# suous/RecNeXt

Measured on AMD Instinct MI355X. Metric: images/sec RecNeXt-M3 224x224 bf16, higher is better.
Workload: dtype bf16

## Files before the change

### include/recnext_amd.h

```cpp
#ifndef RECNEXT_AMD_H
#define RECNEXT_AMD_H

#include <stddef.h>

#ifdef __cplusplus
extern "C" {
#endif

#define RCX_ABI_VERSION 7

enum { RCX_DTYPE_F32 = 0, RCX_DTYPE_BF16 = 1, RCX_DTYPE_F16 = 2 };
enum { RCX_MODE_BILINEAR = 0, RCX_MODE_NEAREST = 1 };
enum { RCX_MAX_LEVEL = 8 };

enum {
    RCX_ERR_BAD_ARG = -1,
    RCX_ERR_UNSUPPORTED = -2,
    RCX_ERR_WORKSPACE = -3
};

int rcx_abi_version(void);
const char* rcx_last_error(void);
void rcx_reload_options(void);

// ... 10 lines not shown
size_t rcx_recconv2d_fwd_workspace_bytes(int N, int C, int H, int W, int level, int k, int dtype);

int rcx_recconv2d_fwd(const void* x, void* y, const float* wpack, const float* bpack,
                      void* workspace, size_t workspace_bytes,
                      int N, int C, int H, int W, int level, int k, int mode, int dtype, void* stream);

int rcx_time_next_launch(void* start_event, void* stop_event);
int rcx_launch_events_pending(void);

size_t rcx_recconv2d_train_saved_bytes(int N, int C, int H, int W, int level, int k);
size_t rcx_recconv2d_bwd_workspace_bytes(int N, int C, int H, int W, int level, int k);
int rcx_recconv2d_fwd_train(const void* x, void* y, const float* wpack, const float* bpack, void* saved, size_t saved_bytes,
                            int N, int C, int H, int W, int level, int k, int mode, int dtype, void* stream);
int rcx_recconv2d_bwd_gy_dtype(int N, int C, int H, int W, int level, int k, int dtype);
const char* rcx_recconv2d_bwd_plan(int N, int C, int H, int W, int level, int k, int dtype);
int rcx_recconv2d_bwd(const void* x, const void* gy, int gy_dtype, const float* wpack, const float* wpack_flipped, const void* saved,
                      void* gx, float* gwpack, float* gbpack, void* const* gw_out, void* const* gb_out, int grad_dtype,
                      void* workspace, size_t workspace_bytes,
                      int N, int C, int H, int W, int level, int k, int mode, int dtype, void* stream);

size_t rcx_recconv2d_bwd_input_workspace_bytes(int N, int C, int H, int W, int level, int k);
int rcx_recconv2d_bwd_input_gy_dtype(int N, int C, int H, int W, int level, int k, int dtype);
const char* rcx_recconv2d_bwd_input_plan(int N, int C, int H, int W, int level, int k, int dtype);
int rcx_recconv2d_bwd_input(const void* gy, int gy_dtype, const float* wpack, const float* wpack_flipped, void* gx,
                            void* workspace, size_t workspace_bytes,
                            int N, int C, int H, int W, int level, int k, int mode, int dtype, void* stream);

int rcx_dwconv2d_fwd(const void* x, void* y, const float* w_kkc, const float* bias,
                     int N, int C, int H, int W, int k, int stride,
                     int in_dtype, int out_dtype, void* stream);

int rcx_dwconv2d_mult2_fwd(const void* x, void* y, const float* w_kkc, const float* bias,
                           int N, int Cin, int H, int W, int k, int stride, int dtype, void* stream);

const char* rcx_upadd_dwconv_fwd_plan(int N, int C, int H, int W, int Hc, int Wc, int k, int mode,
                                      int x_dtype, int coarse_dtype, int out_dtype, int has_coarse);
int rcx_upadd_dwconv_fwd(const void* x, const void* coarse, void* y, const float* w_kkc, const float* bias,
                         int N, int C, int H, int W, int Hc, int Wc, int k, int mode,
                         int x_dtype, int coarse_dtype, int out_dtype, void* stream);

size_t rcx_dwconv2d_bwd_workspace_bytes(int C, int k);
int rcx_dwconv2d_bwd(const void* x, const float* gy, const float* w_kkc, const float* w_flipped_kkc,
                     void* gx, float* gw, float* gb, void* workspace, size_t workspace_bytes,
                     int N, int C, int H, int W, int k, int stride, int x_dtype, void* stream);

size_t rcx_upadd_dwconv_bwd_workspace_bytes(int N, int C, int H, int W, int Hc, int Wc, int k);
int rcx_upadd_dwconv_bwd_gy_dtype(int N, int C, int H, int W, int Hc, int Wc, int k, int dtype);
int rcx_upadd_dwconv_bwd(const void* x, const float* coarse, const void* gy, int gy_dtype, const float* w_kkc, const float* w_flipped_kkc,
                         void* gx, float* gcoarse, float* gw, float* gb, void* workspace, size_t workspace_bytes,
                         int N, int C, int H, int W, int Hc, int Wc, int k, int mode, int dtype, void* stream);

int rcx_dwconv2d_mult2_bwd(const void* x, const float* gy, const float* w_kkc, void* gx, float* gw, float* gb,
                           void* workspace, size_t workspace_bytes, int N, int Cin, int H, int W, int k, int dtype, void* stream);

int rcx_linear_attention_fwd(const void* qpre, const void* kpre, const void* v, const void* pe, void* out,
                             int B, int n, int C, int heads, int dtype, void* stream);
int rcx_linear_attention_pe_fwd(const void* qpre, const void* kpre, const void* v, const float* w_pe_kkc, const float* b_pe, void* out,
                                int B, int H, int W, int C, int heads, int dtype, void* stream);

int rcx_recattn_qkcore_launches(int B, int H, int W, int C, int heads);
size_t rcx_recattn_qkcore_workspace_bytes(int B, int H, int W, int C, int heads);
int rcx_recattn_qkcore_fwd(const float* d, const void* wqk_bf16, const float* bqk, const float* w_pe_kkc, const float* b_pe, float* out,
                           void* workspace, size_t workspace_bytes, int B, int H, int W, int C, int heads, void* stream);

int rcx_recattn_down_qkcore_supported(int B, int H, int W, int C, int heads, int x_dtype);
int rcx_recattn_down_qkcore_fwd(const void* x, const float* w_down_kkc, const float* b_down, const void* wqk_bf16, const float* bqk,
// ... 103 lines not shown
```

### recnext_amd/_lib.py

```python
import ctypes
import os

_HERE = os.path.dirname(os.path.abspath(__file__))
LIB_PATH = os.path.join(_HERE, "lib", "librecnext_amd.so")

DTYPE_F32, DTYPE_BF16, DTYPE_F16 = 0, 1, 2
MODE_BILINEAR, MODE_NEAREST = 0, 1
MODES = {"bilinear": MODE_BILINEAR, "nearest": MODE_NEAREST}
MAX_LEVEL = 8
ERR_BAD_ARG, ERR_UNSUPPORTED, ERR_WORKSPACE = -1, -2, -3
ABI_VERSION = 7

_vp, _i, _sz = ctypes.c_void_p, ctypes.c_int, ctypes.c_size_t

SIGNATURES = {
    "rcx_selftest_d16": (_i, [_vp, _vp, _vp]),
    "rcx_abi_version": (_i, []),
    "rcx_last_error": (ctypes.c_char_p, []),
    "rcx_reload_options": (None, []),
    "rcx_recconv2d_fwd_plan": (ctypes.c_char_p, [_i] * 8),
    "rcx_pack_dw_weight": (_i, [_vp, _vp, _i, _i, _i, _vp]),
    "rcx_pack_bias": (_i, [_vp, _vp, _i, _i, _vp]),
    "rcx_pack_recconv_params": (_i, [_vp, _vp, _vp, _vp, _vp, _i, _i, _i, _i, _vp]),
    "rcx_unpack_recconv_grads": (_i, [_vp, _vp, _i, _i, _i, _vp]),
    "rcx_recconv2d_fwd_workspace_bytes": (_sz, [_i] * 7),
    "rcx_recconv2d_fwd": (_i, [_vp, _vp, _vp, _vp, _vp, _sz] + [_i] * 8 + [_vp]),
    "rcx_time_next_launch": (_i, [_vp, _vp]),
    "rcx_launch_events_pending": (_i, []),
    "rcx_recconv2d_train_saved_bytes": (_sz, [_i] * 6),
    "rcx_recconv2d_bwd_workspace_bytes": (_sz, [_i] * 6),
    "rcx_recconv2d_fwd_train": (_i, [_vp, _vp, _vp, _vp, _vp, _sz] + [_i] * 8 + [_vp]),
    "rcx_recconv2d_bwd_gy_dtype": (_i, [_i] * 7),
    "rcx_recconv2d_bwd_plan": (ctypes.c_char_p, [_i] * 7),
    "rcx_upadd_dwconv_bwd_workspace_bytes": (_sz, [_i] * 7),
    "rcx_upadd_dwconv_bwd_gy_dtype": (_i, [_i] * 8),
    "rcx_upadd_dwconv_bwd": (_i, [_vp, _vp, _vp, _i] + [_vp] * 7 + [_sz] + [_i] * 9 + [_vp]),
    "rcx_recconv2d_bwd": (_i, [_vp, _vp, _i] + [_vp] * 8 + [_i, _vp, _sz] + [_i] * 8 + [_vp]),
    "rcx_recconv2d_bwd_input_workspace_bytes": (_sz, [_i] * 6),
    "rcx_recconv2d_bwd_input_gy_dtype": (_i, [_i] * 7),
    "rcx_recconv2d_bwd_input_plan": (ctypes.c_char_p, [_i] * 7),
    "rcx_recconv2d_bwd_input": (_i, [_vp, _i, _vp, _vp, _vp, _vp, _sz] + [_i] * 8 + [_vp]),
    "rcx_dwconv2d_fwd": (_i, [_vp, _vp, _vp, _vp] + [_i] * 8 + [_vp]),
    "rcx_dwconv2d_mult2_fwd": (_i, [_vp, _vp, _vp, _vp] + [_i] * 7 + [_vp]),
    "rcx_upadd_dwconv_fwd": (_i, [_vp, _vp, _vp, _vp, _vp] + [_i] * 11 + [_vp]),
    "rcx_upadd_dwconv_fwd_plan": (ctypes.c_char_p, [_i] * 12),
    "rcx_linear_attention_pe_fwd": (_i, [_vp] * 6 + [_i] * 6 + [_vp]),
    "rcx_recattn_qkcore_launches": (_i, [_i] * 5),
    "rcx_recattn_qkcore_workspace_bytes": (_sz, [_i] * 5),
    "rcx_recattn_qkcore_fwd": (_i, [_vp] * 7 + [_sz] + [_i] * 5 + [_vp]),
    "rcx_recattn_down_qkcore_supported": (_i, [_i] * 6),
    "rcx_recattn_down_qkcore_fwd": (_i, [_vp] * 8 + [_i] * 6 + [_vp]),
    "rcx_stem_supported": (_i, [_i] * 6),
    "rcx_stem_pack_bytes": (_sz, [_i] * 2),
    "rcx_stem_fwd": (_i, [_vp] * 6 + [_i] * 6 + [_vp]),
    "rcx_stem3_supported": (_i, [_i] * 6),
    "rcx_stem3_pack_bytes": (_sz, [_i] * 2),
    "rcx_stem3_workspace_bytes": (_sz, [_i] * 4),
    "rcx_stem3_fwd": (_i, [_vp] * 9 + [_sz] + [_i] * 6 + [_vp]),
    "rcx_channel_mlp_supported": (_i, [_i] * 4),
    "rcx_channel_mlp_pack_bytes": (_sz, [_i] * 2),
    "rcx_channel_mlp_fwd": (_i, [_vp] * 5 + [_i] * 4 + [_vp]),
    "rcx_recattn2d_fwd_supported": (_i, [_i] * 7),
    "rcx_recattn2d_fwd": (_i, [_vp] * 10 + [_i] * 7 + [_vp]),
    "rcx_dwconv2d_bwd_workspace_bytes": (ctypes.c_size_t, [_i, _i]),
    "rcx_dwconv2d_bwd": (_i, [_vp, _vp, _vp, _vp, _vp, _vp, _vp, _vp, ctypes.c_size_t] + [_i] * 7 + [_vp]),
    "rcx_dwconv2d_mult2_bwd": (_i, [_vp, _vp, _vp, _vp, _vp, _vp, _vp, ctypes.c_size_t] + [_i] * 6 + [_vp]),
    "rcx_linear_attention_fwd": (_i, [_vp, _vp, _vp, _vp, _vp] + [_i] * 5 + [_vp]),
    "rcx_ls_recattn_supported": (_i, [_i] * 7),
    "rcx_ls_recattn_fwd": (_i, [_vp] * 15 + [_i] * 7 + [_vp]),
    "rcx_ls_la3_supported": (_i, [_i] * 7),
    "rcx_ls_la3_fwd": (_i, [_vp] * 11 + [_i] * 7 + [_vp]),
    "rcx_ls_recattn_tiled_supported": (_i, [_i] * 7),
    "rcx_ls_recattn_tiled_workspace_bytes": (_sz, [_i] * 7),
    "rcx_ls_recattn_tiled_fwd": (_i, [_vp] * 16 + [_sz] + [_i] * 7 + [_vp]),
    "rcx_ls_la3_tiled_supported": (_i, [_i] * 7),
    "rcx_ls_la3_tiled_workspace_bytes": (_sz, [_i] * 7),
# ... 59 lines not shown
```

### recnext_amd/csrc/rcx_api.hip

```cpp
#include "../../include/recnext_amd.h"
#include "rcx_opts.h"
#include "rcx_launch.h"

#include <cstdarg>
#include <initializer_list>
#include <cstdio>
#include <cstdlib>

namespace {

thread_local char g_err[512] = "";

int fail(int code, const char* fmt, ...)
{
    va_list ap;
    va_start(ap, fmt);
    vsnprintf(g_err, sizeof(g_err), fmt, ap);
    va_end(ap);
    return code;
}

int hip_fail(hipError_t e, const char* what, const char* prefix = "")
{
    snprintf(g_err, sizeof(g_err), "%s%s: %s", prefix, what, hipGetErrorString(e));
// ... 56 lines not shown

size_t split_bytes(int N, int C, int H, int W) { return 2 * align256(sizeof(float) * (size_t)N * C * (H / 2) * (W / 2)); }

bool use_lanes(int N, int C, int H, int W, int level, int k, int dtype)
{
    return !rcx::opt::hand_kernels_off() && rcx::lanes_applicable(N, C, H, W, level, k, dtype);
}

bool upcpt_everywhere() { return rcx::opt::str(rcx::opt::UPADD_CPT)[0] == 'a'; }

enum StepKernel { STEP_GENERIC, STEP_LANES, STEP_CPT, STEP_CPL14, STEP_CONV5_LANES };

StepKernel pick_dwconv(int N, int C, int H, int W, int k, int stride, int in_dt, int out_dt)
{
    if (rcx::opt::hand_kernels_off()) return STEP_GENERIC;
    if (rcx::down5_cpl7_applicable(N, C, H, W, k, stride, in_dt, out_dt)) return STEP_CPL14;
    const bool lanes_ok = rcx::down5_lanes_applicable(N, C, H, W, k, stride, in_dt, out_dt);
    if (lanes_ok && !upcpt_everywhere() && !(W % 14 != 0 && C % 64 == 0)) return STEP_LANES;
    if (rcx::down5_cpt_applicable(N, C, H, W, k, stride, in_dt, out_dt)) return STEP_CPT;
    if (lanes_ok) return STEP_LANES;
    if (stride == 1 && rcx::conv5_lanes_applicable(N, C, H, W, k, in_dt, out_dt)) return STEP_CONV5_LANES;
    return STEP_GENERIC;
}

StepKernel pick_upadd(int N, int C, int H, int W, int Hc, int Wc, int k, int x_dt, int c_dt, int out_dt, bool has_coarse)
{
    if (rcx::opt::hand_kernels_off()) return STEP_GENERIC;
    if (!has_coarse) return rcx::conv5_lanes_applicable(N, C, H, W, k, x_dt, out_dt) ? STEP_CONV5_LANES : STEP_GENERIC;
    if (rcx::upadd_cpl14_applicable(N, C, H, W, Hc, Wc, k, x_dt, c_dt, out_dt)) return STEP_CPL14;
    const bool lanes_ok = rcx::upadd_lanes_applicable(N, C, H, W, Hc, Wc, k, x_dt, c_dt, out_dt);
    const bool whole = C % 64 == 0 && !(W % 14 != 0 && H < 64);
    if ((whole || !lanes_ok || upcpt_everywhere()) && rcx::upadd_cpt_applicable(N, C, H, W, Hc, Wc, k, x_dt, c_dt, out_dt)) return STEP_CPT;
    return lanes_ok ? STEP_LANES : STEP_GENERIC;
}

enum FwdSchedule { FWD_LANES, FWD_SPLIT, FWD_PLANE, FWD_NESTED, FWD_GENERIC };
FwdSchedule fwd_schedule(int N, int C, int H, int W, int level, int k, int dtype);

bool use_nested(int N, int C, int H, int W, int level, int k, int dtype)
{
    if (rcx::opt::hand_kernels_off() || rcx::opt::off(rcx::opt::NESTED) || level < 1 || k != 5 || (H & 1) || (W & 1)) return false;
    const StepKernel d = pick_dwconv(N, C, H, W, k, 2, dtype, RCX_DTYPE_F32);
    const StepKernel u = pick_upadd(N, C, H, W, H / 2, W / 2, k, dtype, RCX_DTYPE_F32, dtype, true);
    if (d == STEP_GENERIC || u == STEP_GENERIC) return false;
    return fwd_schedule(N, C, H / 2, W / 2, level - 1, k, RCX_DTYPE_F32) != FWD_GENERIC;
}

FwdSchedule fwd_schedule(int N, int C, int H, int W, int level, int k, int dtype)
{
    if (use_lanes(N, C, H, W, level, k, dtype)) return FWD_LANES;
    if (use_split(N, C, H, W, level, k, dtype)) return FWD_SPLIT;
    if (use_plane(N, C, H, W, level, k, dtype)) return FWD_PLANE;
    if (use_nested(N, C, H, W, level, k, dtype)) return FWD_NESTED;
    return FWD_GENERIC;
}

size_t nested_own_bytes(int N, int C, int H, int W) { return 2 * align256(sizeof(float) * (size_t)N * C * (H / 2) * (W / 2)); }

hipError_t step_dwconv(const void* x, void* y, const float* w, const float* b, int N, int C, int H, int W, int k, int stride,
                       int in_dt, int out_dt, hipStream_t s)
{
    switch (pick_dwconv(N, C, H, W, k, stride, in_dt, out_dt)) {
    case STEP_CPL14: return rcx::down5_cpl7(x, y, w, b, N, C, H, in_dt, s);
    case STEP_LANES: return rcx::down5_lanes(x, y, w, b, N, C, H, W, in_dt, out_dt, s);
    case STEP_CPT: return rcx::down5_cpt(x, y, w, b, N, C, H, W, in_dt, out_dt, s);
    case STEP_CONV5_LANES: return rcx::conv5_lanes(x, y, w, b, N, C, H, W, in_dt, s);
// ... 544 lines not shown
    const size_t need = bwd_input_workspace(L, sch.kind);
    if (need && (!workspace || workspace_bytes < need))
        return fail(RCX_ERR_WORKSPACE, "input-backward workspace too small: need %zu bytes, got %zu", need, workspace_bytes);
    if (gy_dtype != RCX_DTYPE_F32 && !(sch.kind != BWD_STEPS && gy_dtype == dtype))
        return fail(RCX_ERR_UNSUPPORTED, "gy of dtype %d: this problem takes float32 (rcx_recconv2d_bwd_input_gy_dtype)", gy_dtype);
    BwdRun B{L, false, "bwd input: "};
    B.gy = gy; B.gx = gx; B.wpack = wpack; B.wflip = wpack_flipped; B.ws = (char*)workspace;
    B.gy_dt = gy_dtype; B.N = N; B.C = C; B.level = level; B.k = k; B.mode = mode; B.dtype = dtype; B.s = (hipStream_t)stream;
    if (sch.kind == BWD_ONE) RCX_TRY(one_launch(B, gy, gy_dtype, gx, 0, H, level, dtype), "fused block", B.prefix);
    else return sch.kind == BWD_TILED ? bwd_tiled(B, sch.m) : bwd_steps(B, sch.m);
    return 0;
}

#undef RCX_TRY

int rcx_dwconv2d_fwd(const void* x, void* y, const float* w_kkc, const float* bias,
                     int N, int C, int H, int W, int k, int stride, int in_dtype, int out_dtype, void* stream)
{
    if (int rc = check_common(x, y, N, C, H, W, k, in_dtype)) return rc;
    if (!known_dtype(out_dtype)) return fail(RCX_ERR_BAD_ARG, "unknown dtype %d", out_dtype);
    if (!w_kkc) return fail(RCX_ERR_BAD_ARG, "null weight");
    if (stride != 1 && stride != 2) return fail(RCX_ERR_UNSUPPORTED, "stride %d not supported (1 or 2)", stride);
    hipError_t e = step_dwconv(x, y, w_kkc, bias, N, C, H, W, k, stride, in_dtype, out_dtype, (hipStream_t)stream);
    return e == hipSuccess ? 0 : hip_fail(e, "rcx_dwconv2d_fwd");
}

int rcx_dwconv2d_mult2_fwd(const void* x, void* y, const float* w_kkc, const float* bias,
                           int N, int Cin, int H, int W, int k, int stride, int dtype, void* stream)
{
    if (int rc = check_common(x, y, N, Cin, H, W, k, dtype)) return rc;
    if (!w_kkc) return fail(RCX_ERR_BAD_ARG, "null weight");
    if (stride != 1 && stride != 2) return fail(RCX_ERR_UNSUPPORTED, "stride %d not supported (1 or 2)", stride);
    hipError_t e;
    const bool lanes_ok = !rcx::opt::hand_kernels_off() && rcx::down_lanes_applicable(N, Cin, H, W, k, stride, dtype);
    const bool tiled_ok = !rcx::opt::hand_kernels_off() && rcx::down7m2_cpt_applicable(N, Cin, H, W, k, stride, dtype);
    if (tiled_ok && (!lanes_ok || H > 64 || W > 64 || (H <= 14 && W <= 14) || upcpt_everywhere()))
        e = rcx::down7m2_cpt(x, y, w_kkc, bias, N, Cin, H, W, dtype, (hipStream_t)stream);
    else if (lanes_ok)
        e = rcx::down_lanes(x, y, w_kkc, bias, N, Cin, H, W, k, stride, dtype, (hipStream_t)stream);
    else
        e = rcx::generic_dwconv_mult2(x, y, w_kkc, bias, N, Cin, H, W, k, stride, dtype, (hipStream_t)stream);
    return e == hipSuccess ? 0 : hip_fail(e, "rcx_dwconv2d_mult2_fwd");
}

const char* rcx_upadd_dwconv_fwd_plan(int N, int C, int H, int W, int Hc, int Wc, int k, int mode, int x_dtype, int coarse_dtype, int out_dtype, int has_coarse)
{
    if (N <= 0 || C <= 0 || H <= 0 || W <= 0 || k <= 0 || (k & 1) == 0) return "invalid";
    static thread_local char desc[160];
    switch (pick_upadd(N, C, H, W, Hc, Wc, k, x_dtype, coarse_dtype, out_dtype, has_coarse != 0)) {
    case STEP_CPL14: return H == 7 ? "upadd_cpl14(k_upadd_cpl7)" : "upadd_cpl14(k_upadd_cpl14)";
    case STEP_CPT: return rcx::upadd_cpt_describe(N, C, H, W, mode == RCX_MODE_NEAREST ? 1 : 0, x_dtype, desc, (int)sizeof(desc)) > 0 ? desc : "upadd_cpt(k_upadd_cpt)";
    case STEP_LANES: return "upadd_lanes(k_upadd_lanes)";
    case STEP_CONV5_LANES: return "conv5_lanes(k_upadd_lanes)";
    default: return "generic";
    }
}

int rcx_upadd_dwconv_fwd(const void* x, const void* coarse, void* y, const float* w_kkc, const float* bias,
                         int N, int C, int H, int W, int Hc, int Wc, int k, int mode,
                         int x_dtype, int coarse_dtype, int out_dtype, void* stream)
{
    if (int rc = check_common(x, y, N, C, H, W, k, x_dtype)) return rc;
    if (!known_dtype(out_dtype)) return fail(RCX_ERR_BAD_ARG, "unknown dtype %d", out_dtype);
    if (!w_kkc) return fail(RCX_ERR_BAD_ARG, "null weight");
    if (mode != RCX_MODE_BILINEAR && mode != RCX_MODE_NEAREST) return fail(RCX_ERR_BAD_ARG, "unknown mode %d", mode);
    if (coarse) {
        if (Hc <= 0 || Wc <= 0) return fail(RCX_ERR_BAD_ARG, "non-positive coarse extent %dx%d", Hc, Wc);
        if (!known_dtype(coarse_dtype)) return fail(RCX_ERR_BAD_ARG, "unknown dtype %d", coarse_dtype);
    }
    hipError_t e = step_upadd(x, coarse, y, w_kkc, bias, N, C, H, W, Hc, Wc, k, mode, x_dtype, coarse_dtype, out_dtype, (hipStream_t)stream);
    return e == hipSuccess ? 0 : hip_fail(e, "rcx_upadd_dwconv_fwd");
}

namespace {

// ... 886 lines not shown
```

### recnext_amd/csrc/rcx_launch.h

```cpp
#pragma once
#include <hip/hip_runtime.h>
#include <hip/hip_ext.h>
#include <stddef.h>

#include <atomic>
#define RCX_MAX_DEVICES 64
#define RCX_SET_LDS_ONCE(kfn, bytes)                                                                                              \
    do {                                                                                                                          \
        static std::atomic<size_t> rcx_lds_set_[RCX_MAX_DEVICES];                                                                 \
        int rcx_dev_ = 0;                                                                                                         \
        if (hipGetDevice(&rcx_dev_) != hipSuccess || rcx_dev_ < 0 || rcx_dev_ >= RCX_MAX_DEVICES) rcx_dev_ = RCX_MAX_DEVICES - 1; \
        if ((size_t)(bytes) > 64 * 1024 && (size_t)(bytes) > rcx_lds_set_[rcx_dev_].load(std::memory_order_acquire)) {            \
            hipError_t rcx_e_ = hipFuncSetAttribute(reinterpret_cast<const void*>(kfn), hipFuncAttributeMaxDynamicSharedMemorySize, (int)(bytes)); \
            if (rcx_e_ != hipSuccess) return rcx_e_;                                                                              \
            if (rcx_dev_ != RCX_MAX_DEVICES - 1) rcx_lds_set_[rcx_dev_].store((size_t)(bytes), std::memory_order_release);        \
        }                                                                                                                         \
    } while (0)

namespace rcx {

struct LaunchEvents { hipEvent_t start = nullptr, stop = nullptr; };
LaunchEvents take_launch_events();
#define RCX_LAUNCH_TIMED(kfn, grid, block, lds, stream, ...)                                                                       \
    do {                                                                                                                           \
// ... 14 lines not shown
hipError_t pack_bias(const void* b, float* dst, int C, int dt, hipStream_t s);
struct PackPtrs { const void* w[10]; const void* b[10]; };
hipError_t pack_params(const PackPtrs& P, float* wpack, float* wflip, float* bpack, int count, int C, int k, int dt, hipStream_t s);
hipError_t unpack_grads(const float* gwpack, const PackPtrs& P, int count, int C, int k, hipStream_t s);

bool plane_applicable(int N, int C, int H, int W, int level, int k, int dtype);
int plane_describe(int N, int C, int H, int W, int level, int k, int dtype, char* buf, int len);
hipError_t plane_recconv(const void* x, void* y, const float* wpack, const float* bpack,
                         int N, int C, int H, int W, int level, int k, int mode, int dtype, hipStream_t s);

bool lanes_applicable(int N, int C, int H, int W, int level, int k, int dtype);
int lanes_describe(int N, int C, int H, int W, int level, int k, int mode, int dtype, char* buf, int len);
hipError_t lanes_recconv(const void* x, void* y, const float* wpack, const float* bpack,
                         int N, int C, int H, int W, int level, int k, int mode, int dtype, hipStream_t s);

hipError_t lanes16_recconv(const void* x, void* y, const float* wpack, const float* bpack,
                           int N, int C, int H, int W, int level, int k, int mode, int dtype, hipStream_t s);


bool cpl14_applicable(int N, int C, int H, int W, int level, int k, int dtype);
bool cpl14_short_applicable(int N, int C, int H, int W, int level, int k, int dtype);
int cpl14_short_describe(int N, int C, int mode, char* buf, int len);
hipError_t cpl14_short_recconv(const void* x, void* y, const float* wpack, const float* bpack, int N, int C, int mode, int dtype, hipStream_t s);
int cpl14_describe(int N, int C, int mode, int dtype, char* buf, int len);
hipError_t cpl14_recconv(const void* x, void* y, const float* wpack, const float* bpack, int N, int C, int mode, int dtype, hipStream_t s,
                         float* saved = nullptr, const size_t* f_off = nullptr, const size_t* c_off = nullptr);

bool upadd_cpt_applicable(int N, int C, int H, int W, int Hc, int Wc, int k, int x_dt, int c_dt, int out_dt);
int upadd_cpt_describe(int N, int C, int H, int W, int mode, int x_dt, char* buf, int len);
hipError_t upadd_cpt(const void* x, const void* coarse, void* y, const float* w, const float* b, int N, int C, int H, int W, int mode,
                     int x_dt, int c_dt, hipStream_t s);
bool down7m2_cpt_applicable(int N, int Cin, int H, int W, int k, int stride, int dtype);
hipError_t down7m2_cpt(const void* x, void* y, const float* w, const float* b, int N, int Cin, int H, int W, int dtype, hipStream_t s);
bool down5_cpt_applicable(int N, int C, int H, int W, int k, int stride, int in_dt, int out_dt);
hipError_t down5_cpt(const void* x, void* y, const float* w, const float* b, int N, int C, int H, int W, int in_dt, int out_dt, hipStream_t s);
bool upadd_cpl14_applicable(int N, int C, int H, int W, int Hc, int Wc, int k, int x_dt, int c_dt, int out_dt);
hipError_t upadd_cpl14(const void* x, const void* coarse, void* y, const float* w, const float* b, int N, int C, int H, int mode, int x_dt, int c_dt,
                       hipStream_t s);
bool down5_cpl7_applicable(int N, int C, int H, int W, int k, int stride, int in_dt, int out_dt);
hipError_t down5_cpl7(const void* x, void* y, const float* w, const float* b, int N, int C, int H, int in_dt, hipStream_t s);

bool cpl7b_applicable(int N, int C, int H, int W, int level, int k, int dtype);
int cpl7b_describe(int N, int C, int mode, char* buf, int len);
hipError_t cpl7b_recconv(const void* x, void* y, const float* wpack, const float* bpack, int N, int C, int mode, int dtype, hipStream_t s,
                         float* saved = nullptr, const size_t* f_off = nullptr, const size_t* c_off = nullptr);

bool cplbwd_applicable(int N, int C, int H, int W, int level, int k, int dtype);
bool cplbwd_split(int N, int C);
hipError_t cplbwd_recconv(const void* x, const void* gy, const float* wpack, const float* wflip, const void* saved,
                          const size_t* f_off, const size_t* c_off, void* gx, float* const* part,
                          int N, int C, int H, int level, int mode, int dtype, hipStream_t s, int gy_dt = 0);

bool cpladj_applicable(int N, int C, int H, int W, int level, int k, int dtype);
hipError_t cpladj_recconv(const void* gy, int gy_dt, const float* wpack, const float* wflip, void* gx, int gx_dt, int N, int C, int H, int mode,
                          hipStream_t s);

bool wgrad_cpl_applicable(int N, int C, int H, int W, int Hc, int Wc, int k, int stride, bool has_coarse);
hipError_t wgrad_cpl(const void* a, int a_dt, const float* coarse, const void* g, int g_dt, float* partial, int N, int C, int H, int mode,
                     hipStream_t s, int* rows_out);

bool wgrad2_cpl_applicable(int N, int C, int H, int W, int Ho, int Wo, int k, int stride, bool has_coarse);
hipError_t wgrad2_cpl(const void* a, int a_dt, const float* g, float* partial, int N, int C, int H, hipStream_t s, int* rows_out);
bool wgrad2m_cpl_applicable(int N, int Cout, int H, int W, int k);
hipError_t wgrad2m_cpl(const void* a, int a_dt, const float* g, float* partial, int N, int Cout, int H, hipStream_t s, int* rows_out);

bool bwd_cpt_applicable(int N, int C, int H, int W, int k);
// ... 140 lines not shown
```

### recnext_amd/csrc/rcx_opts.h

```cpp
#pragma once
#include <stdlib.h>
#include <mutex>
#include <string>

namespace rcx {
namespace opt {

enum Id { FORCE_GENERIC, CPL, CPL14, CPL14_RL, CPT, CPT_CB, CPT16, UPADD_CPL, UPADD_CPT, NESTED, TRAIN_FUSED, BWD_FUSED, WGRAD_CPL, COUNT };

namespace detail {
inline const char* name_of(int i)
{
    static const char* const k[COUNT] = {"RCX_FORCE_GENERIC", "RCX_CPL", "RCX_CPL14", "RCX_CPL14_RL", "RCX_CPT", "RCX_CPT_CB", "RCX_CPT16",
                                         "RCX_UPADD_CPL", "RCX_UPADD_CPT", "RCX_NESTED", "RCX_TRAIN_FUSED", "RCX_BWD_FUSED", "RCX_WGRAD_CPL"};
    return k[i];
}
struct Table {
    std::string val[COUNT];
    std::once_flag once;
    void read()
    {
        for (int i = 0; i < COUNT; ++i) {
            const char* v = getenv(name_of(i));
            val[i] = v ? v : "";
        }
    }
};
inline Table& table() { static Table t; return t; }
}

inline const char* str(Id id)
{
    detail::Table& t = detail::table();
    std::call_once(t.once, [&] { t.read(); });
    return t.val[id].c_str();
}
inline bool off(Id id) { return str(id)[0] == '0'; }
inline bool on(Id id) { const char* v = str(id); return *v && *v != '0'; }
inline int int_or(Id id, int dflt) { const char* v = str(id); return *v ? atoi(v) : dflt; }
inline void reload()
{
    detail::Table& t = detail::table();
    std::call_once(t.once, [&] { t.read(); });
    t.read();
}

inline bool hand_kernels_off() { return on(FORCE_GENERIC); }
// ... 4 lines not shown
```

### recnext_amd/csrc/rcx_upcpt.hip

```cpp
#include "rcx_cpt_kernel.h"
#include "rcx_opts.h"

namespace rcx {
namespace upcpt {

using namespace cpt;

static inline int tile_width(int W, int x_dt) { return (W % 14 != 0 && W % 16 == 0 && x_dt == 1) ? 16 : 14; }

constexpr int NR = 18;

template <int MODE, int TW, int AHEAD> struct Sched {
    static constexpr int NCOL = TW + 4, NCR = TW / 2 + 4, NSTORE = TW;
    static constexpr int c_last = MODE == 0 ? 8 : 7;
    static constexpr bool is_build(int ri) { return MODE == 0 ? (ri & 1) == 1 : ((ri & 1) == 0 && ri >= 2); }
    static constexpr int build_row(int ri) { return MODE == 0 ? (ri - 1) / 2 : (ri - 2) / 2; }
    static constexpr int pending(int kind, int ri_target)
    {
        int seq = 0, xend[NR + AHEAD + 1] = {}, cend[16] = {};
        for (int i = -2; i <= 0; ++i) { seq += NCR; cend[i + 2] = seq; }
        for (int r = 0; r < AHEAD; ++r) { seq += NCOL; xend[r] = seq; }
        if (kind == 0) return seq - cend[1];
        for (int ri = 0; ri < NR; ++ri) {
            if (ri + AHEAD < NR) { seq += NCOL; xend[ri + AHEAD] = seq; }
// ... 591 lines not shown
            for (int i = 0; i < 7; ++i) a[i] = pfma(xr[i + 2], tp[u][2], a[i]);
#pragma unroll
            for (int i = 0; i < 7; ++i) a[i].x = fmaf(xr[i + 3].x, tp[u][3].x, a[i].x);
            if (u == 6) {
                float out[7];
#pragma unroll
                for (int i = 0; i < 7; ++i) out[i] = a[i].x + a[i].y;
                DownSt<TIO>::st(out, yoff, row_desc(ybase, 7 * tr + ot, Ho, Wo * pixo), 0, pixo);
            }
        }
#pragma unroll
        for (int ot = 0; ot < 7; ++ot) if (r - 2 * ot + 3 >= 0 && r - 2 * ot + 3 < 6) pin(facc[ot % 4]);
        CPT_FENCE;
    });
}

template <typename TIO>
static hipError_t launch_down7(const void* x, void* y, const float* w, const float* b, int N, int Cin, int H, int W, hipStream_t s)
{
    const long long units = (long long)N * ((2 * Cin + 63) / 64) * ((H + 13) / 14) * ((W + 13) / 14);
    const dim3 grid((unsigned)((units + 3) / 4)), block(256);
    const int hb = b != nullptr;
    const int pixb = Cin * (int)sizeof(TIO);
#define RCX_GO(PB) hipLaunchKernelGGL((k_down7m2_cpt<PB, TIO>), grid, block, 0, s, (const TIO*)x, (TIO*)y, w, b, N, Cin, H, W, hb)
    if constexpr (sizeof(TIO) == 2) {
        if (pixb == 128) { RCX_GO(128); return hipGetLastError(); }
        if (pixb == 256) { RCX_GO(256); return hipGetLastError(); }
    }
    RCX_GO(0);
#undef RCX_GO
    return hipGetLastError();
}

static inline bool enabled() { return !rcx::opt::off(rcx::opt::UPADD_CPT) && !rcx::opt::hand_kernels_off(); }

template <int MODE, typename TIO, typename TC>
static hipError_t launch(const void* x, const void* coarse, void* y, const float* w, const float* b, int N, int C, int H, int W, hipStream_t s)
{
    const int tw = tile_width(W, std::is_same<TIO, bf16_t>::value ? 1 : 0);
    const long long units = (long long)N * ((C + 63) / 64) * ((H + 13) / 14) * ((W + tw - 1) / tw);
    const dim3 grid((unsigned)((units + 3) / 4)), block(256);
    const int hb = b != nullptr;
    const int pixb = C * (int)sizeof(TIO);
#define RCX_GO(PB, TW) hipLaunchKernelGGL((k_upadd_cpt<MODE, PB, TIO, TC, TW>), grid, block, 0, s, (const TIO*)x, (const TC*)coarse, (TIO*)y, w, b, N, C, H, W, hb)
    if constexpr (std::is_same<TIO, bf16_t>::value) {
        if (tw == 16) {
            if (pixb == 128) RCX_GO(128, 16);
            else if (pixb == 256) RCX_GO(256, 16);
            else RCX_GO(0, 16);
            return hipGetLastError();
        }
    }
    if constexpr (sizeof(TIO) == 2) {
        if (pixb == 128) { RCX_GO(128, 14); return hipGetLastError(); }
        if (pixb == 256) { RCX_GO(256, 14); return hipGetLastError(); }
    }
    RCX_GO(0, 14);
#undef RCX_GO
    return hipGetLastError();
}

}

bool upadd_cpt_applicable(int N, int C, int H, int W, int Hc, int Wc, int k, int x_dt, int c_dt, int out_dt)
{
    if (!upcpt::enabled() || k != 5 || out_dt != x_dt || x_dt < 0 || x_dt > 2 || !(c_dt == x_dt || c_dt == 0)) return false;
// ... 24 lines not shown
bool down5_cpt_applicable(int N, int C, int H, int W, int k, int stride, int in_dt, int out_dt)
{
    if (!upcpt::enabled() || k != 5 || stride != 2 || in_dt < 0 || in_dt > 2 || !(out_dt == in_dt || out_dt == 0)) return false;
    const int tw = upcpt::tile_width(W, in_dt);
    if (N < 1 || C < 1 || (H & 1) || (W & 1) || H < 28 || W < 28) return false;
    const long long img = (long long)H * W * C * 4;
    const long long units = (long long)N * ((C + 63) / 64) * ((H + 13) / 14) * ((W + tw - 1) / tw);
    return img < (1ll << 31) && units < (1ll << 31);
}

hipError_t down5_cpt(const void* x, void* y, const float* w, const float* b, int N, int C, int H, int W, int in_dt, int out_dt, hipStream_t s)
{
    if (in_dt == 1) return out_dt == 1 ? upcpt::launch_down<bf16_t, bf16_t>(x, y, w, b, N, C, H, W, s) : upcpt::launch_down<bf16_t, float>(x, y, w, b, N, C, H, W, s);
    if (in_dt == 2) return out_dt == 2 ? upcpt::launch_down<f16_t, f16_t>(x, y, w, b, N, C, H, W, s) : upcpt::launch_down<f16_t, float>(x, y, w, b, N, C, H, W, s);
    return upcpt::launch_down<float, float>(x, y, w, b, N, C, H, W, s);
}

bool down7m2_cpt_applicable(int N, int Cin, int H, int W, int k, int stride, int dtype)
{
    if (!upcpt::enabled() || k != 7 || stride != 2 || dtype < 0 || dtype > 2) return false;
    if (N < 1 || Cin < 1 || (H & 1) || (W & 1) || H < 14 || W < 14) return false;
    const long long img = (long long)H * W * Cin * 4;
    const long long units = (long long)N * ((2 * Cin + 63) / 64) * ((H + 13) / 14) * ((W + 13) / 14);
    return img < (1ll << 31) && units < (1ll << 31);
}

hipError_t down7m2_cpt(const void* x, void* y, const float* w, const float* b, int N, int Cin, int H, int W, int dtype, hipStream_t s)
{
    if (dtype == 1) return upcpt::launch_down7<bf16_t>(x, y, w, b, N, Cin, H, W, s);
    if (dtype == 2) return upcpt::launch_down7<f16_t>(x, y, w, b, N, Cin, H, W, s);
    return upcpt::launch_down7<float>(x, y, w, b, N, Cin, H, W, s);
}

}
```

### recnext_amd/ops.py

```python
import torch

from . import _lib

_DT = {torch.float32: _lib.DTYPE_F32, torch.bfloat16: _lib.DTYPE_BF16, torch.float16: _lib.DTYPE_F16}


_D16_CHECKED = set()


def selftest_d16(device):
    dev = torch.device(device)
    src = (torch.arange(64, device=dev, dtype=torch.int32) * 517 + 0x1234).to(torch.int16)
    flag = torch.zeros(1, dtype=torch.int32, device=dev)
    with torch.cuda.device(dev):
        rc = _lib.load().rcx_selftest_d16(src.data_ptr(), flag.data_ptr(), _stream(dev))
    _lib.check(rc, "rcx_selftest_d16")
    mask = int(flag.item())
    if mask:
        raise _lib.RcxError(f"D16 self-test failed on {dev} (mask {mask:#x}: bit 0 global_load_short_d16_hi, 1 buffer_load_short_d16_hi, 2 "
                            "ds_read_u16_d16_hi): this device does not zero the other half of a D16-hi load; the 16-bit kernels would return garbage")
    _D16_CHECKED.add(dev.index if dev.index is not None else torch.cuda.current_device())
    return mask


# ... 221 lines not shown
    x = _nhwc(x)
    n, c, h, w = x.shape
    out_dtype = out_dtype or x.dtype
    hc = wc = 0
    cdt = _lib.DTYPE_F32
    if coarse is not None:
        coarse = _nhwc(coarse, "coarse")
        if coarse.shape[0] != n or coarse.shape[1] != c:
            raise ValueError("coarse must share N and C with x")
        hc, wc = coarse.shape[2:]
        cdt = _dt(coarse)
    y = _empty_nhwc(n, c, h, w, out_dtype, x.device)
    with _on(x.device):
        rc = _lib.load().rcx_upadd_dwconv_fwd(x.data_ptr(), coarse.data_ptr() if coarse is not None else None, y.data_ptr(),
                                              w_kkc.data_ptr(), bias.data_ptr() if bias is not None else None,
                                              n, c, h, w, hc, wc, k, _lib.MODES[mode], _dt(x), cdt, _DT[out_dtype],
                                              _stream(x.device))
    _lib.check(rc, "rcx_upadd_dwconv_fwd")
    return y


def dwconv2d_mult2(x, w_kkc, bias=None, k=7, stride=2):
    x = _nhwc(x)
    n, c, h, w = x.shape
    p = k // 2
    ho, wo = (h + 2 * p - k) // stride + 1, (w + 2 * p - k) // stride + 1
    y = _empty_nhwc(n, 2 * c, ho, wo, x.dtype, x.device)
    with _on(x.device):
        rc = _lib.load().rcx_dwconv2d_mult2_fwd(x.data_ptr(), y.data_ptr(), w_kkc.data_ptr(),
                                                bias.data_ptr() if bias is not None else None,
                                                n, c, h, w, k, stride, _dt(x), _stream(x.device))
    _lib.check(rc, "rcx_dwconv2d_mult2_fwd")
    return y


def _conv_out_shape(x, mult, k, stride):
    n, c, h, w = x.shape
    p = k // 2
    return (n, c * mult, (h + 2 * p - k) // stride + 1, (w + 2 * p - k) // stride + 1)


def dwconv2d_backward(x, gy, w_kkc, k, stride, need_input_grad=True, need_bias=False):
    _check_bwd_args("dwconv2d_backward", x, shapes=[("gy", gy, _conv_out_shape(x, 1, k, stride))], packs=[("w_kkc", w_kkc, k * k * x.shape[1])])
    x = _nhwc(x)
    n, c, h, w = x.shape
    gy = _nhwc(gy.to(torch.float32), "grad_output")
    lib = _lib.load()
    wflip = w_kkc.view(k, k, c).flip(0, 1).contiguous()
    gx = _empty_nhwc(n, c, h, w, x.dtype, x.device) if need_input_grad else None
    gw = torch.empty(k * k * c, dtype=torch.float32, device=x.device)
    gb = torch.empty(c, dtype=torch.float32, device=x.device) if need_bias else None
    nbytes = lib.rcx_dwconv2d_bwd_workspace_bytes(c, k)
    ws = torch.empty(max(nbytes, 1), dtype=torch.uint8, device=x.device)
    with _on(x.device):
        rc = lib.rcx_dwconv2d_bwd(x.data_ptr(), gy.data_ptr(), w_kkc.data_ptr(), wflip.data_ptr(),
                                  gx.data_ptr() if gx is not None else None, gw.data_ptr(), gb.data_ptr() if gb is not None else None,
                                  ws.data_ptr(), nbytes, n, c, h, w, k, stride, _dt(x), _stream(x.device))
    _lib.check(rc, "rcx_dwconv2d_bwd")
    return gx, gw, gb


def upadd_dwconv_backward(x, coarse, gy, w_kkc, k=5, mode="nearest", need_input_grad=True, need_coarse_grad=True, need_bias=False):
    _check_bwd_args("upadd_dwconv_backward", x, shapes=[("coarse", coarse, None), ("gy", gy, x.shape)], packs=[("w_kkc", w_kkc, k * k * x.shape[1])])
    x = _nhwc(x)
    coarse = _nhwc(coarse, "coarse")
    if coarse.dtype != torch.float32:
# ... 612 lines not shown
```

Measured before the change: 118,600.

## Add paired-channel kernel for stride-2 multiplier-2 depthwise downsample conv

Adds a new k_down7m2_pair kernel in which each lane computes both output channels of one input channel, using packed f32x2 FMAs against interleaved weight pairs. It is selected by default for 16-bit inputs with Cin a multiple of 64 and spatial size above 14. The aim is to load each input row once for both outputs and halve scalar FMA issue, reducing memory traffic and instruction count in the downsampling layers. It keeps a larger register set (7x7 weight pairs and four accumulator rows), which may lower occupancy. A plan query and an RCX_DOWN_PAIR override are also added.

```diff
diff --git a/include/recnext_amd.h b/include/recnext_amd.h
--- a/include/recnext_amd.h
+++ b/include/recnext_amd.h
@@ -66,6 +66,7 @@
 
 int rcx_dwconv2d_mult2_fwd(const void* x, void* y, const float* w_kkc, const float* bias,
                            int N, int Cin, int H, int W, int k, int stride, int dtype, void* stream);
+const char* rcx_dwconv2d_mult2_fwd_plan(int N, int Cin, int H, int W, int k, int stride, int dtype);
 
 const char* rcx_upadd_dwconv_fwd_plan(int N, int C, int H, int W, int Hc, int Wc, int k, int mode,
                                       int x_dtype, int coarse_dtype, int out_dtype, int has_coarse);
diff --git a/recnext_amd/_lib.py b/recnext_amd/_lib.py
--- a/recnext_amd/_lib.py
+++ b/recnext_amd/_lib.py
@@ -42,6 +42,7 @@
     "rcx_recconv2d_bwd_input": (_i, [_vp, _i, _vp, _vp, _vp, _vp, _sz] + [_i] * 8 + [_vp]),
     "rcx_dwconv2d_fwd": (_i, [_vp, _vp, _vp, _vp] + [_i] * 8 + [_vp]),
     "rcx_dwconv2d_mult2_fwd": (_i, [_vp, _vp, _vp, _vp] + [_i] * 7 + [_vp]),
+    "rcx_dwconv2d_mult2_fwd_plan": (ctypes.c_char_p, [_i] * 7),
     "rcx_upadd_dwconv_fwd": (_i, [_vp, _vp, _vp, _vp, _vp] + [_i] * 11 + [_vp]),
     "rcx_upadd_dwconv_fwd_plan": (ctypes.c_char_p, [_i] * 12),
     "rcx_linear_attention_pe_fwd": (_i, [_vp] * 6 + [_i] * 6 + [_vp]),
diff --git a/recnext_amd/csrc/rcx_api.hip b/recnext_amd/csrc/rcx_api.hip
--- a/recnext_amd/csrc/rcx_api.hip
+++ b/recnext_amd/csrc/rcx_api.hip
@@ -112,6 +112,25 @@
     const bool whole = C % 64 == 0 && !(W % 14 != 0 && H < 64);
     if ((whole || !lanes_ok || upcpt_everywhere()) && rcx::upadd_cpt_applicable(N, C, H, W, Hc, Wc, k, x_dt, c_dt, out_dt)) return STEP_CPT;
     return lanes_ok ? STEP_LANES : STEP_GENERIC;
+}
+
+enum Mult2Kernel { M2_GENERIC, M2_LANES, M2_CPT, M2_PAIR };
+
+bool pair_wins(int Cin, int H, int W, int dtype, Mult2Kernel parent)
+{
+    return (parent == M2_CPT || parent == M2_LANES) && dtype != RCX_DTYPE_F32 && Cin % 64 == 0 && (H > 14 || W > 14);
+}
+
+Mult2Kernel pick_mult2(int N, int Cin, int H, int W, int k, int stride, int dtype)
+{
+    if (rcx::opt::hand_kernels_off()) return M2_GENERIC;
+    const bool lanes_ok = rcx::down_lanes_applicable(N, Cin, H, W, k, stride, dtype);
+    const bool tiled_ok = rcx::down7m2_cpt_applicable(N, Cin, H, W, k, stride, dtype);
+    const Mult2Kernel parent = tiled_ok && (!lanes_ok || H > 64 || W > 64 || (H <= 14 && W <= 14) || upcpt_everywhere()) ? M2_CPT
+                               : lanes_ok ? M2_LANES : M2_GENERIC;
+    const char* sw = rcx::opt::str(rcx::opt::DOWN_PAIR);
+    if (sw[0] == '0' || upcpt_everywhere() || !rcx::down7m2_pair_applicable(N, Cin, H, W, k, stride, dtype)) return parent;
+    return sw[0] == 'a' || pair_wins(Cin, H, W, dtype, parent) ? M2_PAIR : parent;
 }
 
 enum FwdSchedule { FWD_LANES, FWD_SPLIT, FWD_PLANE, FWD_NESTED, FWD_GENERIC };
@@ -722,15 +741,28 @@
     if (!w_kkc) return fail(RCX_ERR_BAD_ARG, "null weight");
     if (stride != 1 && stride != 2) return fail(RCX_ERR_UNSUPPORTED, "stride %d not supported (1 or 2)", stride);
     hipError_t e;
-    const bool lanes_ok = !rcx::opt::hand_kernels_off() && rcx::down_lanes_applicable(N, Cin, H, W, k, stride, dtype);
-    const bool tiled_ok = !rcx::opt::hand_kernels_off() && rcx::down7m2_cpt_applicable(N, Cin, H, W, k, stride, dtype);
-    if (tiled_ok && (!lanes_ok || H > 64 || W > 64 || (H <= 14 && W <= 14) || upcpt_everywhere()))
-        e = rcx::down7m2_cpt(x, y, w_kkc, bias, N, Cin, H, W, dtype, (hipStream_t)stream);
-    else if (lanes_ok)
-        e = rcx::down_lanes(x, y, w_kkc, bias, N, Cin, H, W, k, stride, dtype, (hipStream_t)stream);
-    else
-        e = rcx::generic_dwconv_mult2(x, y, w_kkc, bias, N, Cin, H, W, k, stride, dtype, (hipStream_t)stream);
+    switch (pick_mult2(N, Cin, H, W, k, stride, dtype)) {
+    case M2_PAIR: e = rcx::down7m2_pair(x, y, w_kkc, bias, N, Cin, H, W, dtype, (hipStream_t)stream); break;
+    case M2_CPT: e = rcx::down7m2_cpt(x, y, w_kkc, bias, N, Cin, H, W, dtype, (hipStream_t)stream); break;
+    case M2_LANES: e = rcx::down_lanes(x, y, w_kkc, bias, N, Cin, H, W, k, stride, dtype, (hipStream_t)stream); break;
+    default: e = rcx::generic_dwconv_mult2(x, y, w_kkc, bias, N, Cin, H, W, k, stride, dtype, (hipStream_t)stream); break;
+    }
     return e == hipSuccess ? 0 : hip_fail(e, "rcx_dwconv2d_mult2_fwd");
+}
+
+const char* rcx_dwconv2d_mult2_fwd_plan(int N, int Cin, int H, int W, int k, int stride, int dtype)
+{
+    if (N <= 0 || Cin <= 0 || H <= 0 || W <= 0 || k <= 0 || (k & 1) == 0 || (stride != 1 && stride != 2) || !known_dtype(dtype)) return "invalid";
+    const int pixb = Cin * (dtype == RCX_DTYPE_F32 ? 4 : 2), imm = pixb == 128 || pixb == 256 ? pixb : 0;
+    const Mult2Kernel m = pick_mult2(N, Cin, H, W, k, stride, dtype);
+    switch (m) {
+    case M2_PAIR: return imm == 128 ? "down_pair(k_down7m2_pair<128>)" : imm == 256 ? "down_pair(k_down7m2_pair<256>)" : "down_pair(k_down7m2_pair<0>)";
+    case M2_CPT:
+        if (dtype == RCX_DTYPE_F32) return "down_cpt(k_down7m2_cpt<0>)";
+        return imm == 128 ? "down_cpt(k_down7m2_cpt<128>)" : imm == 256 ? "down_cpt(k_down7m2_cpt<256>)" : "down_cpt(k_down7m2_cpt<0>)";
+    case M2_LANES: return "down_lanes(k_down_lanes)";
+    default: return "generic";
+    }
 }
 
 const char* rcx_upadd_dwconv_fwd_plan(int N, int C, int H, int W, int Hc, int Wc, int k, int mode, int x_dtype, int coarse_dtype, int out_dtype, int has_coarse)
diff --git a/recnext_amd/csrc/rcx_launch.h b/recnext_amd/csrc/rcx_launch.h
--- a/recnext_amd/csrc/rcx_launch.h
+++ b/recnext_amd/csrc/rcx_launch.h
@@ -70,6 +70,8 @@
                      int x_dt, int c_dt, hipStream_t s);
 bool down7m2_cpt_applicable(int N, int Cin, int H, int W, int k, int stride, int dtype);
 hipError_t down7m2_cpt(const void* x, void* y, const float* w, const float* b, int N, int Cin, int H, int W, int dtype, hipStream_t s);
+bool down7m2_pair_applicable(int N, int Cin, int H, int W, int k, int stride, int dtype);
+hipError_t down7m2_pair(const void* x, void* y, const float* w, const float* b, int N, int Cin, int H, int W, int dtype, hipStream_t s);
 bool down5_cpt_applicable(int N, int C, int H, int W, int k, int stride, int in_dt, int out_dt);
 hipError_t down5_cpt(const void* x, void* y, const float* w, const float* b, int N, int C, int H, int W, int in_dt, int out_dt, hipStream_t s);
 bool upadd_cpl14_applicable(int N, int C, int H, int W, int Hc, int Wc, int k, int x_dt, int c_dt, int out_dt);
diff --git a/recnext_amd/csrc/rcx_opts.h b/recnext_amd/csrc/rcx_opts.h
--- a/recnext_amd/csrc/rcx_opts.h
+++ b/recnext_amd/csrc/rcx_opts.h
@@ -6,13 +6,13 @@
 namespace rcx {
 namespace opt {
 
-enum Id { FORCE_GENERIC, CPL, CPL14, CPL14_RL, CPT, CPT_CB, CPT16, UPADD_CPL, UPADD_CPT, NESTED, TRAIN_FUSED, BWD_FUSED, WGRAD_CPL, COUNT };
+enum Id { FORCE_GENERIC, CPL, CPL14, CPL14_RL, CPT, CPT_CB, CPT16, UPADD_CPL, UPADD_CPT, NESTED, TRAIN_FUSED, BWD_FUSED, WGRAD_CPL, DOWN_PAIR, COUNT };
 
 namespace detail {
 inline const char* name_of(int i)
 {
     static const char* const k[COUNT] = {"RCX_FORCE_GENERIC", "RCX_CPL", "RCX_CPL14", "RCX_CPL14_RL", "RCX_CPT", "RCX_CPT_CB", "RCX_CPT16",
-                                         "RCX_UPADD_CPL", "RCX_UPADD_CPT", "RCX_NESTED", "RCX_TRAIN_FUSED", "RCX_BWD_FUSED", "RCX_WGRAD_CPL"};
+                                         "RCX_UPADD_CPL", "RCX_UPADD_CPT", "RCX_NESTED", "RCX_TRAIN_FUSED", "RCX_BWD_FUSED", "RCX_WGRAD_CPL", "RCX_DOWN_PAIR"};
     return k[i];
 }
 struct Table {
diff --git a/recnext_amd/csrc/rcx_upcpt.hip b/recnext_amd/csrc/rcx_upcpt.hip
--- a/recnext_amd/csrc/rcx_upcpt.hip
+++ b/recnext_amd/csrc/rcx_upcpt.hip
@@ -647,6 +647,112 @@
     return hipGetLastError();
 }
 
+template <typename TIO> struct PairSt {
+    static __device__ __forceinline__ void st(const f32x2 (&a)[7], unsigned vo, i32x4 rs, int pixo)
+    {
+        float p[7];
+#pragma unroll
+        for (int i = 0; i < 7; ++i) p[i] = __uint_as_float(pk16<TIO>(a[i].x, a[i].y));
+        DownSt<float>::st(p, vo, rs, 0, pixo);
+    }
+};
+template <> struct PairSt<float> {
+    static __device__ __forceinline__ void st(const f32x2 (&a)[7], unsigned vo, i32x4 rs, int pixo)
+    {
+        int t;
+        asm volatile("s_mov_b32 %[t], 0\n\t" DN_S("buffer_store_dwordx2", 0) DN_N DN_S("buffer_store_dwordx2", 1) DN_N DN_S("buffer_store_dwordx2", 2) DN_N
+                     DN_S("buffer_store_dwordx2", 3) DN_N DN_S("buffer_store_dwordx2", 4) DN_N DN_S("buffer_store_dwordx2", 5) DN_N DN_S("buffer_store_dwordx2", 6)
+                     : [t] "=&s"(t)
+                     : [p0] "v"(a[0]), [p1] "v"(a[1]), [p2] "v"(a[2]), [p3] "v"(a[3]), [p4] "v"(a[4]), [p5] "v"(a[5]), [p6] "v"(a[6]),
+                       [vo] "v"(vo), [rs] "s"(rs), [pix] "s"(pixo) : "scc", "memory");
+    }
+};
+
+template <int PIXB, typename TIO>
+__global__ __launch_bounds__(256, 2) void k_down7m2_pair(const TIO* __restrict__ x, TIO* __restrict__ y, const float* __restrict__ w, const float* __restrict__ bias,
+                                                         int N, int Cin, int H, int W, int has_bias)
+{
+    constexpr int ESZ = (int)sizeof(TIO), AHEAD = 1;
+    using S = SchedDown7<AHEAD>;
+    const int Co = 2 * Cin, nb = (Cin + 63) / 64, TR = (H + 13) / 14, TCn = (W + 13) / 14, Ho = H / 2, Wo = W / 2;
+    const int pix = PIXB ? PIXB : Cin * ESZ, pixo = 2 * pix;
+    const unsigned total = (unsigned)N * nb * TR * TCn;
+    const int lane = (int)(threadIdx.x & 63);
+    const unsigned upp = (unsigned)(TR * TCn);
+    const unsigned wg = (upp & 3u) == 0 ? xcd_workgroup(blockIdx.x, upp >> 2, total / upp) : blockIdx.x;
+    const unsigned unit = __builtin_amdgcn_readfirstlane(wg * 4 + (threadIdx.x >> 6));
+    if (unit >= total) return;
+    const int tc = (int)(unit % (unsigned)TCn);
+    unsigned q = unit / (unsigned)TCn;
+    const int tr = (int)(q % (unsigned)TR);
+    q /= (unsigned)TR;
+    const int cb = (int)(q % (unsigned)nb), n = (int)(q / (unsigned)nb);
+    const int c = cb * 64 + lane;
+    const bool cvalid = c < Cin;
+    const int cc = cvalid ? c : Cin - 1;
+    const unsigned OOB = 0x80000000u;
+    const unsigned long long xbase = (unsigned long long)(reinterpret_cast<const char*>(x) + (size_t)n * H * W * pix);
+    const unsigned long long ybase = (unsigned long long)(reinterpret_cast<char*>(y) + (size_t)n * Ho * Wo * pixo);
+    const unsigned voffM = (unsigned)((14 * tc) * pix + cc * ESZ);
+    const unsigned voffL = voffM - 3u * (unsigned)pix;
+    const unsigned voffR = voffM + 14u * (unsigned)pix;
+    auto load_row = [&](uint32_t (&raw)[20], int r) { row_load7<TIO, PIXB>(raw, voffL, voffM, voffR, row_desc(xbase, 14 * tr + r, H, W * pix), 0, pix); };
+    uint32_t raw[NR7][20];
+    sfor<AHEAD>([&](auto rc) { load_row(raw[decltype(rc)::value], -3 + decltype(rc)::value); });
+    const __amdgpu_buffer_rsrc_t wsrc = __builtin_amdgcn_make_buffer_rsrc((void*)w, 0, 49 * Co * 4, 0x00020000);
+    const __amdgpu_buffer_rsrc_t bsrc = __builtin_amdgcn_make_buffer_rsrc((void*)bias, 0, has_bias ? Co * 4 : 0, 0x00020000);
+    f32x2 tp[7][7];
+#pragma unroll
+    for (int u = 0; u < 7; ++u) {
+#pragma unroll
+        for (int v = 0; v < 7; ++v) tp[u][v] = __builtin_bit_cast(f32x2, __builtin_amdgcn_raw_buffer_load_b64(wsrc, cc * 8, (u * 7 + v) * Co * 4, 0));
+    }
+    f32x2 b0 = __builtin_bit_cast(f32x2, __builtin_amdgcn_raw_buffer_load_b64(bsrc, cc * 8, 0, 0));
+#pragma unroll
+    for (int u = 0; u < 7; ++u) pin(tp[u]);
+    pin(b0);
+    const unsigned yoff = cvalid ? (unsigned)((7 * tc) * pixo + c * 2 * ESZ) : OOB;
+    f32x2 facc[4][7];
+    sfor<NR7>([&](auto rc) {
+        constexpr int ri = decltype(rc)::value, r = ri - 3;
+        if constexpr (ri + AHEAD < NR7) load_row(raw[ri + AHEAD], r + AHEAD);
+        pin_row20<S::cap(S::pending(ri))>(raw[ri]);
+        float xv[20];
+#pragma unroll
+        for (int j = 0; j < 20; ++j) xv[j] = raw_f32<TIO>(raw[ri][j]);
+#pragma unroll
+        for (int ot = 0; ot < 7; ++ot) {
+            const int u = r - 2 * ot + 3;
+            if (u < 0 || u > 6) continue;
+            f32x2(&a)[7] = facc[ot % 4];
+#pragma unroll
+            for (int v = 0; v < 7; ++v) {
+#pragma unroll
+                for (int i = 0; i < 7; ++i) a[i] = pfma(splat(xv[2 * i + v]), tp[u][v], (u == 0 && v == 0) ? b0 : a[i]);
+            }
+            if (u == 6) PairSt<TIO>::st(a, yoff, row_desc(ybase, 7 * tr + ot, Ho, Wo * pixo), pixo);
+        }
+#pragma unroll
+        for (int ot = 0; ot < 7; ++ot) if (r - 2 * ot + 3 >= 0 && r - 2 * ot + 3 < 6) pin(facc[ot % 4]);
+        CPT_FENCE;
+    });
+}
+
+template <typename TIO>
+static hipError_t launch_down7_pair(const void* x, void* y, const float* w, const float* b, int N, int Cin, int H, int W, hipStream_t s)
+{
+    const long long units = (long long)N * ((Cin + 63) / 64) * ((H + 13) / 14) * ((W + 13) / 14);
+    const dim3 grid((unsigned)((units + 3) / 4)), block(256);
+    const int hb = b != nullptr;
+    const int pixb = Cin * (int)sizeof(TIO);
+#define RCX_GO(PB) hipLaunchKernelGGL((k_down7m2_pair<PB, TIO>), grid, block, 0, s, (const TIO*)x, (TIO*)y, w, b, N, Cin, H, W, hb)
+    if (pixb == 128) { RCX_GO(128); return hipGetLastError(); }
+    if (pixb == 256) { RCX_GO(256); return hipGetLastError(); }
+    RCX_GO(0);
+#undef RCX_GO
+    return hipGetLastError();
+}
+
 static inline bool enabled() { return !rcx::opt::off(rcx::opt::UPADD_CPT) && !rcx::opt::hand_kernels_off(); }
 
 template <int MODE, typename TIO, typename TC>
@@ -737,4 +843,18 @@
     return upcpt::launch_down7<float>(x, y, w, b, N, Cin, H, W, s);
 }
 
-}
+bool down7m2_pair_applicable(int N, int Cin, int H, int W, int k, int stride, int dtype)
+{
+    if (!down7m2_cpt_applicable(N, Cin, H, W, k, stride, dtype)) return false;
+    const long long units = (long long)N * ((Cin + 63) / 64) * ((H + 13) / 14) * ((W + 13) / 14);
+    return units < (1ll << 31);
+}
+
+hipError_t down7m2_pair(const void* x, void* y, const float* w, const float* b, int N, int Cin, int H, int W, int dtype, hipStream_t s)
+{
+    if (dtype == 1) return upcpt::launch_down7_pair<bf16_t>(x, y, w, b, N, Cin, H, W, s);
+    if (dtype == 2) return upcpt::launch_down7_pair<f16_t>(x, y, w, b, N, Cin, H, W, s);
+    return upcpt::launch_down7_pair<float>(x, y, w, b, N, Cin, H, W, s);
+}
+
+}
diff --git a/recnext_amd/ops.py b/recnext_amd/ops.py
--- a/recnext_amd/ops.py
+++ b/recnext_amd/ops.py
@@ -277,6 +277,10 @@
                                                 n, c, h, w, k, stride, _dt(x), _stream(x.device))
     _lib.check(rc, "rcx_dwconv2d_mult2_fwd")
     return y
+
+
+def dwconv2d_mult2_plan(n, c, h, w, dtype, k=7, stride=2):
+    return _lib.load().rcx_dwconv2d_mult2_fwd_plan(n, c, h, w, k, stride, _DT[dtype]).decode()
 
 
 def _conv_out_shape(x, mult, k, stride):
```

After: 119,500 (median of 6 runs). About the same (+0.8%).
